# AdamStelmaszczyk/Distributed-BA3C

Measured on AMD Instinct MI355X. Metric: BA3C train-step samples/sec, 84x84x4 frames, batch 32 & 2048, at 1/2/4/8 GPUs, higher is better.
Workload: dtype f32; 1 GPU; configs[2]/[3]: BA3C train step (fwd+bwd+clip+Adam) B=2048/GPU, fc_neurons=512, fc_splits=1, A=4; global_batch=2048, per_gpu_batch=2048, fc_neurons=512, fc_splits=1, num_actions=4, parallelism=dp1, backup_workers=0

## Files before the change

distributed-ba3c_amd/csrc/ba3c_capi.hip:

```cpp
#include <hip/hip_runtime.h>
#include <dlfcn.h>
#include <rccl/rccl.h>

#include <cmath>
#include <cstdio>
#include <cstring>
#include <optional>
#include <string>
#include <type_traits>
#include <vector>

#include "../../include/ba3c.h"
#include "ba3c_band6.h"
#include "ba3c_boxing.h"
#include "ba3c_breakout.h"
#include "ba3c_conv.h"
#include "ba3c_conv3.h"
#include "ba3c_duel.h"
#include "ba3c_envview.h"
#include "ba3c_gemm6.h"
#include "ba3c_launch.h"
#include "ba3c_multi.h"
#include "ba3c_plan.h"
#include "ba3c_problems.h"
// ... 800 lines not shown
                                                          dim3(B * C2D::G::NBANDS), wa, wg, 0, dim3(0, 1, 1), h,
                                                          BA3C_K_CONV2_DGRAD)));
    }
    h->merged[BA3C_K_CONV2_DGRAD] |= 1u << BA3C_K_CONV2_WGRAD;
    return reduce_wgrad6<W2>(h, wa, (int)wg.x, dW2);
  }

  int conv1() {
    if (!pl.split) {
      const WgradPlan p = plan_wgrad(800, 32, B * 1296, 128, 32);
      ConvWgrad<false, 40, 40, 32, 5, 5, 32, true> g{w.p0, w.dp1, w.c1, w.part_1, 1.0f, p.M, p.N, p.K, p.kchunk};
      CHECK((launch_gemm<128, 32, 4, 1>(h, ws, BA3C_K_CONV1_WGRAD, g, p.S)));
      CHECK(conv_reduce(p.M, p.N, p.S, 1, 32, 32, w.part_1));
      ConvDgrad<40, 40, 32, 5, 5, 32, true> d{w.dp1, w.c1, param(h->idx_conv[1]), w.dp0, B * 1600, 32, 800, 0};
      return launch_gemm<128, 32, 4, 1>(h, s, BA3C_K_CONV1_DGRAD, d, 1);
    }
    const Wg6Args wa = wa1();
    float* dW1 = grad(h->idx_conv[1]);
    const int P = pl.conv1_slabs;
    const BandArgs ba{w.dp1, w.c1, w.wt + WT_C1D, w.dp0, nullptr, nullptr, B};
    const SplitIO io{AM_DP1, WJ_C1D, AM_DP0};
    if (pl.mj) {
      CHECK((launch_multi<true, Band6Job<typename LY::C1D>, Wg6Job<W1>>(
          s, band6_args<typename LY::C1D>(h, ba, w, WT_C1D, io), dim3(B * LY::C1D::G::NBANDS), wa,
          wgrad6_grid<W1>(P, B))));
      h->merged[BA3C_K_CONV1_DGRAD] |= 1u << BA3C_K_CONV1_WGRAD;
      return reduce_wgrad6<W1>(h, wa, P, dW1);
    }
    if (pl.conv1_wgrad == Conv1Wgrad::whole) {
      {
        ProbeScope ps(h, ws, BA3C_K_CONV1_WGRAD);
        hipLaunchKernelGGL(wgrad6w_kernel<typename LY::W1W>, dim3(P), dim3(256), 0, ws, wa);
      }
      HIP_TRY(hipGetLastError());
      CHECK(reduce_wgrad6<W1>(h, wa, P, dW1));
    } else if (pl.conv1_wgrad == Conv1Wgrad::wgrad6) {
      CHECK(launch_wgrad6<W1>(h, ws, BA3C_K_CONV1_WGRAD, wa, P, dW1));
    }
    return launch_band6<typename LY::C1D>(h, s, BA3C_K_CONV1_DGRAD, ba, w, WT_C1D, io, pl.ring_dgrad);
  }

  int conv0() {
    ReduceMap mp{};
    mp.kind = 0;
    mp.N = 32;
    mp.cin = CH;
    mp.cinpad = 16;
    mp.dst = grad(h->idx_conv[0]);
    if (pl.split && CH == 4) {
      const int P = pl.conv0_slabs;
      const Conv0WArgs a0{state, w.dp0, w.c0, w.part0, B, w.am(AM_DP0, h)};
      if (pl.conv1_wgrad == Conv1Wgrad::pair0) {
        const Wg6Args wa = wa1();
        {
          ProbeScope ps(h, s, BA3C_K_CONV0_WGRAD);
          HIP_TRY(launch_wgrad01_pair(s, wa, pl.conv1_slabs, a0, P));
        }
        h->merged[BA3C_K_CONV0_WGRAD] |= 1u << BA3C_K_CONV1_WGRAD;
        CHECK(reduce_wgrad6<W1>(h, wa, pl.conv1_slabs, grad(h->idx_conv[1])));
      } else {
        ProbeScope ps(h, s, BA3C_K_CONV0_WGRAD);
        HIP_TRY(launch_conv0s_wgrad(dim3(P), s, a0));
      }
      mp.M = Conv0W<2>::M;
      return add_reduce(h, w.part0, P, mp);
    }
    const WgradPlan p = plan_wgrad(25 * CH, 32, B * 6400, 128, 32);
    ConvWgrad<true, 84, 84, CH, 5, 5, 32, true> g{state, w.dp0, w.c0, w.part0, 1.0f / 255.0f, p.M, p.N, p.K, p.kchunk};
    CHECK((launch_gemm<128, 32, 4, 1>(h, s, BA3C_K_CONV0_WGRAD, g, p.S)));
    mp.M = p.M;
    return add_reduce(h, w.part0, p.S, mp);
  }
};

struct PpoArgs {
  const float* rows;
  float* ratio;
  float clip_eps;
  bool ext = false;
  float vclip_eps = 0.f;
  unsigned flags = 0;
};

template <int LOSS>
void launch_heads(hipStream_t s, int B, const HeadsArgsOf<LOSS>& a) {
  const int F = a.F;
  const dim3 g((B + 3) / 4), t(256);
  if (a.A == 4 && F <= 128 && F > 64) hipLaunchKernelGGL((heads_kernel<2, FC_SPLIT, 4, LOSS>), g, t, 0, s, a);
  else if (a.A == 4 && F <= 512 && F > 256) hipLaunchKernelGGL((heads_kernel<8, FC_SPLIT, 4, LOSS>), g, t, 0, s, a);
  else if (F <= 64) hipLaunchKernelGGL((heads_kernel<1, FC_SPLIT, 0, LOSS>), g, t, 0, s, a);
  else if (F <= 128) hipLaunchKernelGGL((heads_kernel<2, FC_SPLIT, 0, LOSS>), g, t, 0, s, a);
  else if (F <= 256) hipLaunchKernelGGL((heads_kernel<4, FC_SPLIT, 0, LOSS>), g, t, 0, s, a);
  else if (F <= 512) hipLaunchKernelGGL((heads_kernel<8, FC_SPLIT, 0, LOSS>), g, t, 0, s, a);
  else hipLaunchKernelGGL((heads_kernel<0, FC_SPLIT, 0, LOSS>), g, t, 0, s, a);
}

int run_heads(ba3c_handle* h, hipStream_t s, const float* prm, const Workspace& w, int B,
              const int64_t* action, const float* R, float beta, float explore, bool train,
              float* probs, float* probsT, float* value, double* scalars = nullptr,
              bool defer_scalars = false, const PpoArgs* ppo = nullptr) {
  HeadsArgsPpoExt a{};
  if (ppo) {
    a.rows = reinterpret_cast<const float4*>(ppo->rows);
    a.ratio = ppo->ratio;
    a.clip_eps = ppo->clip_eps;
    a.vclip_eps = ppo->vclip_eps;
    a.flags = ppo->flags;
  }
  a.fcpart = w.fcpart;
// ... 142 lines not shown
}

template <class Rules>
static int env_view(void* stream, const int32_t* game, int32_t n_envs, const int32_t* sel, int32_t n_sel,
                    const uint8_t* palette, const uint8_t* hud, int32_t scale, uint8_t* out) {
  if (!game || !palette || !out) return fail(BA3C_ERR_INVALID, "null game / palette / out pointer");
  if (n_envs < 1 || n_sel < 1) return fail(BA3C_ERR_INVALID, "n_envs and n_sel must be >= 1");
  if (scale < 1 || scale > VIEW_MAX_SCALE) return fail(BA3C_ERR_INVALID, "scale must be in [1, 8]");
  if (!check_ptr(game) || ((reinterpret_cast<uintptr_t>(out) | reinterpret_cast<uintptr_t>(sel) |
                            reinterpret_cast<uintptr_t>(hud)) & 3))
    return fail(BA3C_ERR_INVALID, "game must be 16-byte and sel / hud / out 4-byte aligned");
  hipStream_t s = static_cast<hipStream_t>(stream);
  ViewArgs a{game, n_envs, sel, palette, hud, scale, out};
  hipLaunchKernelGGL(env_view_kernel<Rules>, dim3(n_sel), dim3(256), 0, s, a);
  HIP_TRY(hipGetLastError());
  return BA3C_OK;
}

extern "C" {

int ba3c_version(void) { return 1; }

const char* ba3c_last_error(void) { return g_err.c_str(); }

int ba3c_create(const ba3c_config* cfg, ba3c_handle** out) {
  if (!cfg || !out) return fail(BA3C_ERR_INVALID, "null argument");
  const ba3c_config& c = *cfg;
  if (c.channels != 4 && c.channels != 12)
    return fail(BA3C_ERR_INVALID, "channels must be 4 or 12 (FRAME_HISTORY * --channels)");
  if (c.num_actions < 1 || c.num_actions >= MAXA)
    return fail(BA3C_ERR_INVALID, "num_actions must be in [1, 31]");
  if (c.max_batch < 1 || c.max_batch > kMaxBatch)
    return fail(BA3C_ERR_INVALID, "max_batch must be in [1, 16384]");
  const int splits = c.replace_with_conv ? c.fc_splits : c.ps;
  if (splits < 1 || c.fc_neurons < 4 || c.fc_neurons % splits != 0 || (c.fc_neurons / splits) % 4 != 0)
    return fail(BA3C_ERR_INVALID, "fc_neurons must be a multiple of 4*fc_splits (or 4*ps)");
  Switches sw;
  struct Switch {
    const char* name;
    const char* digits;
    void (*set)(Switches&, int);
  };
  const Switch switches[] = {
      {"BA3C_GENERIC", "01", [](Switches& w, int v) { w.generic = v != 0; }},
      {"BA3C_C1PAIR", "02", [](Switches& w, int v) { w.c1pair = v; }},
      {"BA3C_SCALARS_RIDE", "01", [](Switches& w, int v) { w.scalars_ride = v != 0; }},
      {"BA3C_OVERLAP", "012", [](Switches& w, int v) { w.overlap = v; }},
      {"BA3C_MULTI", "01", [](Switches& w, int v) { w.multi = v != 0; }},
      {"BA3C_MULTI_BIG", "0123", [](Switches& w, int v) { w.multi_big = v; }},
      {"BA3C_FUSED_UPDATE", "01", [](Switches& w, int v) { w.fused_update = v != 0; }},
      {"BA3C_RING", "01", [](Switches& w, int v) { w.ring = v != 0; }},
      {"BA3C_CHAIN", "01", [](Switches& w, int v) { w.chain = v != 0; }},
      {"BA3C_FWD01", "01", [](Switches& w, int v) { w.fwd01 = v != 0; }},
  };
  for (const Switch& k : switches) {
    const char* e = getenv(k.name);
    if (!e) continue;
    if (!e[0] || e[1] || !strchr(k.digits, e[0]))
      return fail(BA3C_ERR_INVALID, std::string(k.name) + "=" + e + ": expected one digit of " + k.digits);
    k.set(sw, e[0] - '0');
  }
  ba3c_handle* h = new ba3c_handle();
  h->cfg = c;
  h->sw = sw;
  h->band = h->g6 = !sw.generic;
  {
    int dev = 0, n = 0;
    if (hipGetDevice(&dev) == hipSuccess &&
        hipDeviceGetAttribute(&n, hipDeviceAttributeMultiprocessorCount, dev) == hipSuccess && n > 0)
      h->cus = n;
  }

  const int F = c.fc_neurons, per = F / splits;
  h->per = per;
  int64_t off = 0;
  auto add = [&](const std::string& name, std::initializer_list<int> shape) {
    TensorDesc d;
    d.name = name;
    d.offset = off;
    d.ndim = (int)shape.size();
    int64_t n = 1;
    int i = 0;
    for (int v : shape) {
      d.shape[i++] = v;
      n *= v;
    }
    for (; i < 4; ++i) d.shape[i] = 0;
    d.numel = n;
    h->tensors.push_back(d);
    off = align64(off + n);
    return (int)h->tensors.size() - 1;
  };
  h->idx_conv[0] = add("conv0/W", {5, 5, 16, 32});
  h->idx_conv[1] = add("conv1/W", {5, 5, 32, 32});
  h->idx_conv[2] = add("conv2/W", {5, 5, 32, 64});
  h->idx_conv[3] = add("conv3/W", {3, 3, 64, 64});
  h->idx_fc1 = -1;
  for (int i = 0; i < splits; ++i) {
    int t;
    if (c.replace_with_conv) {
      t = add("fc1_" + std::to_string(i) + "/W", {5, 5, 64, per});
    } else {
      t = add("fc1_" + std::to_string(i) + "/W", {1600, per});
      add("fc1_" + std::to_string(i) + "/b", {per});
    }
    if (i == 0) h->idx_fc1 = t;
// ... 685 lines not shown
```

distributed-ba3c_amd/csrc/ba3c_conv0.hip:

```cpp
#include <hip/hip_runtime.h>

#define BA3C_SHARED_KERNELS 0

#include "ba3c_launch.h"
#include "ba3c_split.h"
#include "ba3c_band6.h"
#include "ba3c_wgrad6.h"

namespace ba3c {

hipError_t launch_conv0s_fwd(dim3 grid, hipStream_t s, const Conv0SArgs& a) {
  hipLaunchKernelGGL(conv0s_fwd_kernel, grid, dim3(256), 0, s, a);
  return hipGetLastError();
}

__global__ void __launch_bounds__(256) __attribute__((amdgpu_waves_per_eu(2)))
wgrad01_pair_kernel(const Wg6Args a1, const Conv0WArgs a0, int g1, int g0) {
  constexpr int B1 = wgrad6w_lds_bytes<Conv1W6W>(), B0 = Conv0W<2>::ALLOC_U4 * 16;
  __shared__ uint4 lds[(B1 > B0 ? B1 : B0) / 16];
  __shared__ uint32_t red4[4];
  const int b = blockIdx.x;
  if (b < g1) {
    wgrad6w_body<Conv1W6W>(a1, b, g1, reinterpret_cast<char*>(lds), red4);
  } else {
    conv0s_wgrad_body<2>(a0, b - g1, g0, lds, red4);
  }
}

hipError_t launch_wgrad01_pair(hipStream_t s, const Wg6Args& a1, int g1, const Conv0WArgs& a0, int g0) {
  hipLaunchKernelGGL(wgrad01_pair_kernel, dim3(g1 + g0), dim3(256), 0, s, a1, a0, g1, g0);
  return hipGetLastError();
}

constexpr int FWD01_CONV0_PRIO = 2;

__device__ __forceinline__ void fwd01_handoff() {
  __builtin_amdgcn_fence(__ATOMIC_RELEASE, "workgroup");
  __syncthreads();
  __builtin_amdgcn_fence(__ATOMIC_ACQUIRE, "workgroup");
}

template <bool TRAIN>
__global__ void __launch_bounds__(256) __attribute__((amdgpu_waves_per_eu(2)))
fwd01_kernel(const Conv0SArgs a0, const Band6Args a1) {
  using L1 = Conv1FLay;
  constexpr int B0 = conv0s_fwd_lds_bytes(), B1 = L1::LDS_BYTES;
  __shared__ uint4 lds4[(B0 > B1 ? B0 : B1) / 16];
  char* lds = reinterpret_cast<char*>(lds4);
  const int gx = gridDim.x, ipw = (a0.batch + gx - 1) / gx;
  const int img0 = min(a0.batch, (int)blockIdx.x * ipw), img1 = min(a0.batch, img0 + ipw);
  constexpr size_t X_IMG = (size_t)Conv0S::HS * Conv0S::WS * Conv0S::C;
  constexpr size_t P0_IMG = (size_t)(Conv0S::HO / 2) * (Conv0S::WO / 2) * Conv0S::COUT;
  constexpr size_t P1_IMG = (size_t)(L1::G::HO / 2) * (L1::G::WO / 2) * L1::G::COUT;
  for (int img = img0; img < img1; ++img) {
    {
      Conv0SArgs s = a0;
      s.x += img * X_IMG;
      s.out += img * P0_IMG;
      if (TRAIN) s.out_code += img * P0_IMG;
      s.amax_out += img;
      s.batch = 1;
      int z = 0;
      asm volatile("" : "+v"(z));
      s.wb += __builtin_amdgcn_readfirstlane(z);
      __builtin_amdgcn_s_setprio(FWD01_CONV0_PRIO);
      conv0s_fwd_body_t<TRAIN, true>(s, 0, 1, lds);
      __builtin_amdgcn_s_setprio(0);
    }
    fwd01_handoff();
    {
      Band6Args s = a1;
      s.src += img * P0_IMG;
      s.out += img * P1_IMG;
      if (TRAIN) s.out_code += img * P1_IMG;
      s.amax_in += img;
      s.amax_out += img;
      s.batch = 1;
      band6r_body<L1, false, true>(s, 0, 1, lds);
    }
    fwd01_handoff();
  }
}

// ... 13 lines not shown
```

distributed-ba3c_amd/csrc/ba3c_launch.h:

```cpp
#pragma once
#include <hip/hip_runtime.h>

namespace ba3c {

struct Conv0SArgs;
struct Conv0WArgs;
struct Wg6Args;
struct Band6Args;

hipError_t launch_conv0s_fwd(dim3 grid, hipStream_t s, const Conv0SArgs& a);
hipError_t launch_fwd01(int grid, hipStream_t s, const Conv0SArgs& a0, const Band6Args& a1);
hipError_t launch_conv0s_wgrad(dim3 grid, hipStream_t s, const Conv0WArgs& a);
hipError_t launch_wgrad01_pair(hipStream_t s, const Wg6Args& a1, int g1, const Conv0WArgs& a0, int g0);

}
```

distributed-ba3c_amd/csrc/ba3c_plan.h:

```cpp
#pragma once
#include <algorithm>

namespace ba3c {

constexpr int SMALL_B = 128;
constexpr int OVERLAP_B = 128;
static_assert(OVERLAP_B <= SMALL_B, "multi-job conv2 input gradient is the small-batch geometry");
constexpr int WG_P1 = 512;
constexpr int W6_P1 = 256, W6_P2 = 128;
constexpr int W1_NBANDS = 9;
constexpr int C0F_NBANDS = 5;
constexpr int C0W_NBANDS = 10;
#ifndef BA3C_C1W_BPW
#define BA3C_C1W_BPW 3
#endif
inline int conv1_wgrad_p(int B) { return std::max(64, std::min(W6_P1, B * W1_NBANDS / BA3C_C1W_BPW)); }
constexpr int W6W_MIN_B = 512, W6W_P = 512;
static_assert(W6W_P <= WG_P1, "conv1 partial slabs: the allocation covers WG_P1 slabs");
inline bool conv1_pair_geometry(int B, int cus) { return B >= 2 * W6W_MIN_B && B % cus == 0 && cus <= WG_P1; }
inline int conv1_w6w_p(int B, int cus) { return conv1_pair_geometry(B, cus) ? cus : std::min(W6W_P, B); }
constexpr int FW_P0S = 512;
inline int conv0_fwd_p(int B) { return std::min(FW_P0S, B * C0F_NBANDS); }
constexpr int C3W_P = 256;
inline int conv3_wgrad_p(int B, int cus) { return std::min(B, std::min(C3W_P, cus)); }
constexpr int WG_P0S = 512;
inline int conv0_wgrad_p(int B, int cus) {
  return conv1_pair_geometry(B, cus) ? cus : std::min(WG_P0S, B * C0W_NBANDS);
}
inline int conv1_slab_count(int B, int cus) {
  return B >= W6W_MIN_B ? conv1_w6w_p(B, cus) : std::min(conv1_wgrad_p(B), B * W1_NBANDS);
}
inline bool ring_batch(int B, int cus) {
  const int pr = 2 * cus;
  return B >= pr && (B % pr == 0 || B >= 8 * pr);
}

struct Switches {
  bool generic = false;
  int c1pair = 2;
  bool scalars_ride = true;
  int overlap = 2;
  bool multi = true;
  int multi_big = 3;
  bool fused_update = true;
  bool ring = true;
  bool chain = true;
  bool fwd01 = true;
};

enum class Conv1Wgrad {
  gemm,
  wgrad6,
  whole,
  pair0,
};

struct LaunchPlan {
  bool split = true;
  bool prep_multi = false;
  bool ring_fwd = false;
  bool fwd01 = false;
  bool conv2_small = false;
  bool big = false;
  bool mj = false;
  bool mj_fc = false;
  bool fc1_big_tiles = false;
  bool mj_c2 = false;
  bool side_stream = false;
  bool ring_dgrad = false;
  Conv1Wgrad conv1_wgrad = Conv1Wgrad::gemm;
  int conv1_slabs = 0, conv0_slabs = 0, conv3_slabs = 0;
};

inline LaunchPlan plan_launches(const Switches& sw, int B, int channels, int cus, bool train) {
  LaunchPlan p;
  p.split = !sw.generic;
  const bool c4 = channels == 4, small = B <= OVERLAP_B, ring = p.split && sw.ring && ring_batch(B, cus);
  p.prep_multi = p.split && sw.multi && small && c4;
  p.ring_fwd = ring;
  p.fwd01 = ring && c4 && !p.prep_multi && sw.fwd01;
  p.conv2_small = p.split && B <= SMALL_B;
  if (!train) return p;
  const bool mjok = p.split && sw.multi && sw.overlap != 1 && c4;
  p.big = !small;
  p.mj = mjok && small;
  p.mj_fc = p.mj || (mjok && (sw.multi_big & 1));
  p.fc1_big_tiles = p.mj_fc && p.big;
  p.mj_c2 = !p.mj && mjok && (sw.multi_big & 2);
  p.side_stream = !p.mj && (sw.overlap == 1 || (sw.overlap == 2 && small));
  p.ring_dgrad = ring;
  if (!p.split) p.conv1_wgrad = Conv1Wgrad::gemm;
  else if (sw.ring && conv1_pair_geometry(B, cus) && sw.c1pair == 2 && c4) p.conv1_wgrad = Conv1Wgrad::pair0;
  else if (B >= W6W_MIN_B) p.conv1_wgrad = Conv1Wgrad::whole;
  else p.conv1_wgrad = Conv1Wgrad::wgrad6;
  p.conv1_slabs = conv1_slab_count(B, cus);
  p.conv0_slabs = c4 ? conv0_wgrad_p(B, cus) : 0;
  p.conv3_slabs = conv3_wgrad_p(B, cus);
  return p;
}

}
```

distributed-ba3c_amd/csrc/ba3c_small.h:

```cpp
#pragma once
#include "ba3c_problems.h"

namespace ba3c {

constexpr int MAXA = 32;
constexpr int NTERMS = 8;
constexpr int MAXT = 48;
constexpr int UPD_CHUNK = 4096;
static_assert(UPD_CHUNK % 256 == 0, "whole elements per thread");
constexpr int FC_SPLIT_MAX = 16;

__device__ __forceinline__ void st_agent(float* p, float v) {
  __hip_atomic_store(p, v, __ATOMIC_RELAXED, __HIP_MEMORY_SCOPE_AGENT);
}
__device__ __forceinline__ float ld_agent(const float* p) {
  return __hip_atomic_load(const_cast<float*>(p), __ATOMIC_RELAXED, __HIP_MEMORY_SCOPE_AGENT);
}
__device__ __forceinline__ unsigned long long ld_agent(const unsigned long long* p) {
  return __hip_atomic_load(const_cast<unsigned long long*>(p), __ATOMIC_RELAXED, __HIP_MEMORY_SCOPE_AGENT);
}

constexpr int LOSS_A3C = 0, LOSS_PPO = 1, LOSS_PPO_EXT = 2;
struct HeadsArgs {
  float* h;
  const float* piW;
  const float* pib;
  const float* vW;
  const float* vb;
  const int64_t* action;
  const float* R;
  float* probs;
  float* probsT;
  float* value;
  float* dzv;
  float* dh;
  float* terms;
  int B, F, A, train, legacy;
  float beta, explore, invB;
  const float* fcpart;
  int fc_split, per, wstride;
  const float* fc_w1;
  unsigned long long* relu_count;
  unsigned long long* done;
  double* scalars;
};
struct HeadsArgsPpo : HeadsArgs {
  const float4* rows;
  float* ratio;
  float clip_eps;
};
constexpr unsigned PPO_ADV_FROM_ROW = 1u;
struct HeadsArgsPpoExt : HeadsArgsPpo {
  float vclip_eps;
  unsigned flags;
// ... 326 lines not shown
    __shared__ int last;
    __builtin_amdgcn_s_waitcnt(0);
    __syncthreads();
    if (threadIdx.x == 0) last = atomicAdd(p.done, 1ull) == (unsigned long long)(nblk - 1);
    __syncthreads();
    if (last) {
      scalars_block(p.terms, p.B, p.beta, p.relu_count, p.scalars);
      if (threadIdx.x == 0) *p.done = 0ull;
    }
  }
}

template <int FCH, int NZ, int AT = 0, int LOSS = LOSS_A3C>
__global__ void __launch_bounds__(256) heads_kernel(const HeadsArgsOf<LOSS> p) {
  heads_body<FCH, NZ, AT, LOSS>(p, blockIdx.x, gridDim.x);
}

__device__ __forceinline__ double block_sum_d(double v, double* red) {
  const int lane = threadIdx.x & 63, wv = threadIdx.x >> 6;
  v = wave_sum_d(v);
  __syncthreads();
  if (lane == 0) red[wv] = v;
  __syncthreads();
  return ((red[0] + red[1]) + red[2]) + red[3];
}

__global__ void __launch_bounds__(256) ppo_norm_adv_kernel(float4* rows, int n, double* stats) {
  __shared__ double red[4];
  const int t = threadIdx.x;
  double s = 0.0;
  for (int i = t; i < n; i += 256) {
    const float4 r = rows[i];
    s += (double)r.x - (double)r.y;
  }
  const double mean = block_sum_d(s, red) / (double)n;
  double q = 0.0;
  for (int i = t; i < n; i += 256) {
    const float4 r = rows[i];
    const double d = ((double)r.x - (double)r.y) - mean;
    q += d * d;
  }
  const double sd = sqrt(block_sum_d(q, red) / (double)n);
  const double inv = sd + 1e-8;
  for (int i = t; i < n; i += 256) {
    const float4 r = rows[i];
    reinterpret_cast<float*>(rows + i)[3] = (float)((((double)r.x - (double)r.y) - mean) / inv);
  }
  if (stats && t == 0) {
    stats[0] = mean;
    stats[1] = sd;
  }
}

struct ReduceMap {
  int kind;
  int M, N;
  int cin, cinpad;
  int per, wstride;
  int A;
  float* dst;
  float* dst_pib;
  float* dst_vW;
  float* dst_vb;
};

__device__ __forceinline__ void grad_store(float* p, float v) { *p = v; }

__device__ __forceinline__ void reduce_store(const ReduceMap& mp, int m, int n, float v) {
  if (mp.kind == 0) {
    const int kk = m / mp.cin, c = m - kk * mp.cin;
    grad_store(mp.dst + ((size_t)kk * mp.cinpad + c) * mp.N + n, v);
  } else if (mp.kind == 1) {
    const int s = n / mp.per, fl = n - s * mp.per;
    grad_store(mp.dst + (size_t)s * mp.wstride + (size_t)m * mp.per + fl, v);
  } else {
    const int F = mp.M - 1;
    if (m < F) {
      if (n < mp.A) grad_store(mp.dst + (size_t)m * mp.A + n, v);
      else if (n == mp.A) grad_store(mp.dst_vW + m, v);
    } else {
      if (n < mp.A) grad_store(mp.dst_pib + n, v);
      else if (n == mp.A) grad_store(mp.dst_vb, v);
    }
  }
}

#ifndef BA3C_RED_GROUPS
#define BA3C_RED_GROUPS 4
#endif
constexpr int RED_G = BA3C_RED_GROUPS;
static_assert(RED_G >= 1 && RED_G <= 16, "reduction groups");

template <int NG>
__device__ __forceinline__ float red_sum(const float (*red)[64], int lane) {
  float v = red[0][lane];
#pragma unroll
  for (int z = 1; z < NG; ++z) v += red[z][lane];
  return v;
}

__global__ void __launch_bounds__(64 * RED_G) wgrad_reduce_kernel(const float* __restrict__ part, int S,
                                                                  const ReduceMap mp) {
  __shared__ float red[RED_G][64];
  const int lane = threadIdx.x & 63, zg = threadIdx.x >> 6;
  const int MN = mp.M * mp.N;
  const int o = blockIdx.x * 64 + lane;
  float s = 0.f;
  if (o < MN) {
    int z = zg;
    for (; z + 7 * RED_G < S; z += 8 * RED_G) {
      float a[8];
#pragma unroll
      for (int u = 0; u < 8; ++u) a[u] = part[(size_t)(z + RED_G * u) * MN + o];
#pragma unroll
      for (int u = 0; u < 8; ++u) s += a[u];
    }
    for (; z < S; z += RED_G) s += part[(size_t)z * MN + o];
  }
  red[zg][lane] = s;
  __syncthreads();
  if (zg == 0 && o < MN) reduce_store(mp, o / mp.N, o % mp.N, red_sum<RED_G>(red, lane));
}

constexpr int MAX_RJOBS = 8;
struct ReduceJobs {
  int n;
  const float* part[MAX_RJOBS];
  int S[MAX_RJOBS];
  ReduceMap mp[MAX_RJOBS];
  int blk0[MAX_RJOBS + 1];
  int vec[MAX_RJOBS];
};

__host__ __device__ inline bool reduce_vec_ok(const ReduceMap& mp) {
  return mp.kind != 2 && mp.N % 4 == 0 && (mp.kind == 0 || mp.per % 4 == 0);
}

__device__ __forceinline__ int reduce_out_size(const ReduceMap& mp) {
  return mp.kind == 0 ? (mp.M / mp.cin) * mp.cinpad * mp.N : mp.M * mp.N;
}

template <int NG>
__device__ __forceinline__ void wgrad_reduce_body(const ReduceJobs& jobs, int b, char* lds) {
  float4 (*red4)[64] = reinterpret_cast<float4 (*)[64]>(lds);
  float (*red)[64] = reinterpret_cast<float (*)[64]>(lds);
  int j = 0;
  while (j + 1 < jobs.n && jobs.blk0[j + 1] <= b) ++j;
  const ReduceMap& mp = jobs.mp[j];
  const float* __restrict__ part = jobs.part[j];
  const int S = jobs.S[j];
  const int lane = threadIdx.x & 63, zg = threadIdx.x >> 6;
  const int MN = mp.M * mp.N;
  if (jobs.vec[j]) {
    const int o = ((b - jobs.blk0[j]) * 64 + lane) * 4;
    const int NO = reduce_out_size(mp);
    int po = o;
    if (mp.kind == 0 && mp.cinpad != mp.cin && o < NO) {
      const int n = o % mp.N, r = o / mp.N, kk = r / mp.cinpad, c = r - kk * mp.cinpad;
      po = c < mp.cin ? (kk * mp.cin + c) * mp.N + n : -1;
    }
    float4 sv = make_float4(0.f, 0.f, 0.f, 0.f);
    if (o < NO && po >= 0) {
      const float4* __restrict__ p4 = reinterpret_cast<const float4*>(part);
      const int MN4 = MN / 4, q = po / 4;
      int z = zg;
      for (; z + 7 * NG < S; z += 8 * NG) {
        float4 a[8];
#pragma unroll
        for (int u = 0; u < 8; ++u) a[u] = p4[(size_t)(z + NG * u) * MN4 + q];
#pragma unroll
        for (int u = 0; u < 8; ++u) {
          sv.x += a[u].x;
          sv.y += a[u].y;
          sv.z += a[u].z;
          sv.w += a[u].w;
        }
      }
      for (; z < S; z += NG) {
        const float4 a = p4[(size_t)z * MN4 + q];
        sv.x += a.x;
        sv.y += a.y;
        sv.z += a.z;
        sv.w += a.w;
      }
    }
    red4[zg][lane] = sv;
    __syncthreads();
    if (zg == 0 && o < NO) {
      float4 v = red4[0][lane];
#pragma unroll
      for (int z = 1; z < NG; ++z) {
        const float4 r = red4[z][lane];
        v.x += r.x;
        v.y += r.y;
        v.z += r.z;
        v.w += r.w;
      }
      if (po < 0) v = make_float4(0.f, 0.f, 0.f, 0.f);
      float* dst;
      if (mp.kind == 0) {
        dst = mp.dst + o;
      } else {
        const int m = o / mp.N, n = o % mp.N, sidx = n / mp.per, fl = n - sidx * mp.per;
        dst = mp.dst + (size_t)sidx * mp.wstride + (size_t)m * mp.per + fl;
      }
      *reinterpret_cast<float4*>(dst) = v;
    }
    return;
  }
  const int o = (b - jobs.blk0[j]) * 64 + lane;
  const int NO = reduce_out_size(mp);
  int po = o;
  if (mp.kind == 0 && mp.cinpad != mp.cin && o < NO) {
    const int n = o % mp.N, r = o / mp.N, kk = r / mp.cinpad, c = r - kk * mp.cinpad;
    po = c < mp.cin ? (kk * mp.cin + c) * mp.N + n : -1;
  }
  float s = 0.f;
  if (o < NO && po >= 0) {
    int z = zg;
    for (; z + 7 * NG < S; z += 8 * NG) {
      float a[8];
#pragma unroll
      for (int u = 0; u < 8; ++u) a[u] = part[(size_t)(z + NG * u) * MN + po];
#pragma unroll
      for (int u = 0; u < 8; ++u) s += a[u];
    }
    for (; z < S; z += NG) s += part[(size_t)z * MN + po];
  }
  red[zg][lane] = s;
  __syncthreads();
  if (zg == 0 && o < NO) {
    const float v = red_sum<NG>(red, lane);
    if (mp.kind == 0) grad_store(mp.dst + o, po >= 0 ? v : 0.f);
    else reduce_store(mp, o / mp.N, o % mp.N, v);
  }
}

__global__ void __launch_bounds__(64 * RED_G) wgrad_reduce_all_kernel(const ReduceJobs jobs) {
  __shared__ float4 red4[RED_G][64];
  wgrad_reduce_body<RED_G>(jobs, blockIdx.x, reinterpret_cast<char*>(red4));
}

struct TensorTable {
  int n;
  int nchunks;
  long long off[MAXT];
  int numel[MAXT];
  int chunk0[MAXT + 1];
};

__device__ __forceinline__ int table_find(const TensorTable& tt, int b) {
  int lo = 0, hi = tt.n - 1;
  while (lo < hi) {
    const int mid = (lo + hi + 1) >> 1;
    if (tt.chunk0[mid] <= b) lo = mid;
    else hi = mid - 1;
  }
  return lo;
}

__device__ __forceinline__ float block_sum_256(float v, float* red) {
  v = wave_sum_f(v);
  const int w = threadIdx.x >> 6;
  if ((threadIdx.x & 63) == 0) red[w] = v;
  __syncthreads();
  const float r = (red[0] + red[1]) + (red[2] + red[3]);
  __syncthreads();
  return r;
}

__global__ void __launch_bounds__(256) sumsq_kernel(const float* __restrict__ g, const TensorTable tt,
                                                    float* __restrict__ part, int cbase) {
  __shared__ float red[4];
  const int b = blockIdx.x + cbase;
  const int t = table_find(tt, b);
  const int c = b - tt.chunk0[t];
  const int beg = c * UPD_CHUNK;
  const int end = min(tt.numel[t], beg + UPD_CHUNK);
  const float* gt = g + tt.off[t];
  float s = 0.f;
  for (int i = beg + threadIdx.x; i < end; i += 256) s = fmaf(gt[i], gt[i], s);
  s = block_sum_256(s, red);
  if (threadIdx.x == 0) part[b] = s;
}

__device__ __forceinline__ float clip_factor(const TensorTable& tt, int t, const float* part) {
  float ss = 0.f;
  for (int b = tt.chunk0[t] + (int)(threadIdx.x & 63); b < tt.chunk0[t + 1]; b += 64) ss += part[b];
// ... 349 lines not shown
```

Measured before the change: 1.223 million samples/s.

## Ride pending wgrad partial reductions as extra workgroups in the conv0/conv1 wgrad pair launch

Already-queued split-K partial-sum reduction jobs (rjobs) are run inside the conv0/conv1 wgrad pair kernel, using one extra workgroup per CU, instead of in a later separate reduce launch. The pending job list is emptied so it is not reduced twice. The riders use new multi-block vectorized reduce bodies that sum several output blocks per workgroup with deeper unrolling. The aim is to drop a kernel launch and hide reduction bandwidth behind the compute-bound wgrad work, at the cost of extra workgroups competing with the pair kernel for CUs and LDS. This relies on the queued jobs' partial buffers being ready before the launch, which holds on the same stream.

After: 1.229 million samples/s (median of 6 runs). No clear change (+0.5%).

```diff
diff --git a/distributed-ba3c_amd/csrc/ba3c_capi.hip b/distributed-ba3c_amd/csrc/ba3c_capi.hip
--- a/distributed-ba3c_amd/csrc/ba3c_capi.hip
+++ b/distributed-ba3c_amd/csrc/ba3c_capi.hip
@@ -876,9 +876,12 @@
       const Conv0WArgs a0{state, w.dp0, w.c0, w.part0, B, w.am(AM_DP0, h)};
       if (pl.conv1_wgrad == Conv1Wgrad::pair0) {
         const Wg6Args wa = wa1();
+        const ReduceJobs ride = h->rjobs;
+        const int gr = pl.reduce_ride && ws == s && ride.n ? h->cus : 0;
+        if (gr) h->rjobs.n = 0;
         {
           ProbeScope ps(h, s, BA3C_K_CONV0_WGRAD);
-          HIP_TRY(launch_wgrad01_pair(s, wa, pl.conv1_slabs, a0, P));
+          HIP_TRY(launch_wgrad01_pair(s, wa, pl.conv1_slabs, a0, P, &ride, gr));
         }
         h->merged[BA3C_K_CONV0_WGRAD] |= 1u << BA3C_K_CONV1_WGRAD;
         CHECK(reduce_wgrad6<W1>(h, wa, pl.conv1_slabs, grad(h->idx_conv[1])));
@@ -1127,6 +1130,7 @@
       {"BA3C_RING", "01", [](Switches& w, int v) { w.ring = v != 0; }},
       {"BA3C_CHAIN", "01", [](Switches& w, int v) { w.chain = v != 0; }},
       {"BA3C_FWD01", "01", [](Switches& w, int v) { w.fwd01 = v != 0; }},
+      {"BA3C_REDUCE_RIDE", "01", [](Switches& w, int v) { w.reduce_ride = v != 0; }},
   };
   for (const Switch& k : switches) {
     const char* e = getenv(k.name);
diff --git a/distributed-ba3c_amd/csrc/ba3c_conv0.hip b/distributed-ba3c_amd/csrc/ba3c_conv0.hip
--- a/distributed-ba3c_amd/csrc/ba3c_conv0.hip
+++ b/distributed-ba3c_amd/csrc/ba3c_conv0.hip
@@ -3,6 +3,7 @@
 #define BA3C_SHARED_KERNELS 0
 
 #include "ba3c_launch.h"
+#include "ba3c_reduce.h"
 #include "ba3c_split.h"
 #include "ba3c_band6.h"
 #include "ba3c_wgrad6.h"
@@ -14,21 +15,62 @@
   return hipGetLastError();
 }
 
+static_assert(64 * RED_G == 256, "a reduce rider is a workgroup of the pair launch");
+
+constexpr int RIDE_KW = 8, RIDE_UW = 2, RIDE_KD = 2, RIDE_UD = 16, RIDE_DEEP_S = 16 * RED_G;
+
+__device__ __forceinline__ int ride_unit_blocks(const ReduceJobs& rj, int j) {
+  return !rj.vec[j] ? 1 : rj.S[j] >= RIDE_DEEP_S ? RIDE_KD : RIDE_KW;
+}
+
+__device__ __forceinline__ void reduce_ride_body(const ReduceJobs& rj, int r, int gr, char* lds) {
+  int total = 0;
+  for (int j = 0; j < rj.n; ++j) {
+    const int kb = ride_unit_blocks(rj, j);
+    total += (rj.blk0[j + 1] - rj.blk0[j] + kb - 1) / kb;
+  }
+  for (int unit = r; unit < total; unit += gr) {
+    int j = rj.n - 1, u = unit, kb, nu;
+    for (;; --j) {
+      kb = ride_unit_blocks(rj, j);
+      nu = (rj.blk0[j + 1] - rj.blk0[j] + kb - 1) / kb;
+      if (u < nu || j == 0) break;
+      u -= nu;
+    }
+    const int b = u * kb, nblk = min(kb, rj.blk0[j + 1] - rj.blk0[j] - b);
+    if (!rj.vec[j]) {
+      wgrad_reduce_body<RED_G>(rj, rj.blk0[j] + b, lds);
+      __syncthreads();
+    } else if (kb == RIDE_KD) {
+      wgrad_reduce_vec_blocks<RED_G, RIDE_KD, RIDE_UD>(rj, j, b, nblk, lds);
+    } else {
+      wgrad_reduce_vec_blocks<RED_G, RIDE_KW, RIDE_UW>(rj, j, b, nblk, lds);
+    }
+  }
+}
+
 __global__ void __launch_bounds__(256) __attribute__((amdgpu_waves_per_eu(2)))
-wgrad01_pair_kernel(const Wg6Args a1, const Conv0WArgs a0, int g1, int g0) {
+wgrad01_pair_kernel(const Wg6Args a1, const Conv0WArgs a0, int g1, int g0, const ReduceJobs rj) {
   constexpr int B1 = wgrad6w_lds_bytes<Conv1W6W>(), B0 = Conv0W<2>::ALLOC_U4 * 16;
+  constexpr int BR = (RIDE_KW > RIDE_KD ? RIDE_KW : RIDE_KD) * RED_G * 64 * (int)sizeof(float4);
+  static_assert(BR <= (B1 > B0 ? B1 : B0), "the riders' scratch fits the pair's LDS array");
   __shared__ uint4 lds[(B1 > B0 ? B1 : B0) / 16];
   __shared__ uint32_t red4[4];
   const int b = blockIdx.x;
   if (b < g1) {
     wgrad6w_body<Conv1W6W>(a1, b, g1, reinterpret_cast<char*>(lds), red4);
+  } else if (b < g1 + g0) {
+    conv0s_wgrad_body<2>(a0, b - g1, g0, lds, red4);
   } else {
-    conv0s_wgrad_body<2>(a0, b - g1, g0, lds, red4);
+    reduce_ride_body(rj, b - g1 - g0, (int)gridDim.x - g1 - g0, reinterpret_cast<char*>(lds));
   }
 }
 
-hipError_t launch_wgrad01_pair(hipStream_t s, const Wg6Args& a1, int g1, const Conv0WArgs& a0, int g0) {
-  hipLaunchKernelGGL(wgrad01_pair_kernel, dim3(g1 + g0), dim3(256), 0, s, a1, a0, g1, g0);
+hipError_t launch_wgrad01_pair(hipStream_t s, const Wg6Args& a1, int g1, const Conv0WArgs& a0, int g0,
+                               const ReduceJobs* rj, int gr) {
+  static const ReduceJobs none{};
+  if (!rj || rj->n == 0) gr = 0;
+  hipLaunchKernelGGL(wgrad01_pair_kernel, dim3(g1 + g0 + gr), dim3(256), 0, s, a1, a0, g1, g0, gr ? *rj : none);
   return hipGetLastError();
 }
 
diff --git a/distributed-ba3c_amd/csrc/ba3c_launch.h b/distributed-ba3c_amd/csrc/ba3c_launch.h
--- a/distributed-ba3c_amd/csrc/ba3c_launch.h
+++ b/distributed-ba3c_amd/csrc/ba3c_launch.h
@@ -7,10 +7,12 @@
 struct Conv0WArgs;
 struct Wg6Args;
 struct Band6Args;
+struct ReduceJobs;
 
 hipError_t launch_conv0s_fwd(dim3 grid, hipStream_t s, const Conv0SArgs& a);
 hipError_t launch_fwd01(int grid, hipStream_t s, const Conv0SArgs& a0, const Band6Args& a1);
 hipError_t launch_conv0s_wgrad(dim3 grid, hipStream_t s, const Conv0WArgs& a);
-hipError_t launch_wgrad01_pair(hipStream_t s, const Wg6Args& a1, int g1, const Conv0WArgs& a0, int g0);
+hipError_t launch_wgrad01_pair(hipStream_t s, const Wg6Args& a1, int g1, const Conv0WArgs& a0, int g0,
+                               const ReduceJobs* rj, int gr);
 
 }
diff --git a/distributed-ba3c_amd/csrc/ba3c_plan.h b/distributed-ba3c_amd/csrc/ba3c_plan.h
--- a/distributed-ba3c_amd/csrc/ba3c_plan.h
+++ b/distributed-ba3c_amd/csrc/ba3c_plan.h
@@ -46,6 +46,7 @@
   bool ring = true;
   bool chain = true;
   bool fwd01 = true;
+  bool reduce_ride = true;
 };
 
 enum class Conv1Wgrad {
@@ -69,6 +70,7 @@
   bool side_stream = false;
   bool ring_dgrad = false;
   Conv1Wgrad conv1_wgrad = Conv1Wgrad::gemm;
+  bool reduce_ride = false;
   int conv1_slabs = 0, conv0_slabs = 0, conv3_slabs = 0;
 };
 
@@ -93,6 +95,7 @@
   else if (sw.ring && conv1_pair_geometry(B, cus) && sw.c1pair == 2 && c4) p.conv1_wgrad = Conv1Wgrad::pair0;
   else if (B >= W6W_MIN_B) p.conv1_wgrad = Conv1Wgrad::whole;
   else p.conv1_wgrad = Conv1Wgrad::wgrad6;
+  p.reduce_ride = sw.reduce_ride && p.conv1_wgrad == Conv1Wgrad::pair0 && !p.side_stream;
   p.conv1_slabs = conv1_slab_count(B, cus);
   p.conv0_slabs = c4 ? conv0_wgrad_p(B, cus) : 0;
   p.conv3_slabs = conv3_wgrad_p(B, cus);
diff --git a/distributed-ba3c_amd/csrc/ba3c_reduce.h b/distributed-ba3c_amd/csrc/ba3c_reduce.h
--- /dev/null
+++ b/distributed-ba3c_amd/csrc/ba3c_reduce.h
@@ -0,0 +1,246 @@
+#pragma once
+#include <hip/hip_runtime.h>
+
+namespace ba3c {
+
+struct ReduceMap {
+  int kind;
+  int M, N;
+  int cin, cinpad;
+  int per, wstride;
+  int A;
+  float* dst;
+  float* dst_pib;
+  float* dst_vW;
+  float* dst_vb;
+};
+
+__device__ __forceinline__ void grad_store(float* p, float v) { *p = v; }
+
+__device__ __forceinline__ void reduce_store(const ReduceMap& mp, int m, int n, float v) {
+  if (mp.kind == 0) {
+    const int kk = m / mp.cin, c = m - kk * mp.cin;
+    grad_store(mp.dst + ((size_t)kk * mp.cinpad + c) * mp.N + n, v);
+  } else if (mp.kind == 1) {
+    const int s = n / mp.per, fl = n - s * mp.per;
+    grad_store(mp.dst + (size_t)s * mp.wstride + (size_t)m * mp.per + fl, v);
+  } else {
+    const int F = mp.M - 1;
+    if (m < F) {
+      if (n < mp.A) grad_store(mp.dst + (size_t)m * mp.A + n, v);
+      else if (n == mp.A) grad_store(mp.dst_vW + m, v);
+    } else {
+      if (n < mp.A) grad_store(mp.dst_pib + n, v);
+      else if (n == mp.A) grad_store(mp.dst_vb, v);
+    }
+  }
+}
+
+#ifndef BA3C_RED_GROUPS
+#define BA3C_RED_GROUPS 4
+#endif
+constexpr int RED_G = BA3C_RED_GROUPS;
+static_assert(RED_G >= 1 && RED_G <= 16, "reduction groups");
+
+template <int NG>
+__device__ __forceinline__ float red_sum(const float (*red)[64], int lane) {
+  float v = red[0][lane];
+#pragma unroll
+  for (int z = 1; z < NG; ++z) v += red[z][lane];
+  return v;
+}
+
+constexpr int MAX_RJOBS = 8;
+struct ReduceJobs {
+  int n;
+  const float* part[MAX_RJOBS];
+  int S[MAX_RJOBS];
+  ReduceMap mp[MAX_RJOBS];
+  int blk0[MAX_RJOBS + 1];
+  int vec[MAX_RJOBS];
+};
+
+__host__ __device__ inline bool reduce_vec_ok(const ReduceMap& mp) {
+  return mp.kind != 2 && mp.N % 4 == 0 && (mp.kind == 0 || mp.per % 4 == 0);
+}
+
+__device__ __forceinline__ int reduce_out_size(const ReduceMap& mp) {
+  return mp.kind == 0 ? (mp.M / mp.cin) * mp.cinpad * mp.N : mp.M * mp.N;
+}
+
+template <int NG>
+__device__ __forceinline__ void wgrad_reduce_body(const ReduceJobs& jobs, int b, char* lds) {
+  float4 (*red4)[64] = reinterpret_cast<float4 (*)[64]>(lds);
+  float (*red)[64] = reinterpret_cast<float (*)[64]>(lds);
+  int j = 0;
+  while (j + 1 < jobs.n && jobs.blk0[j + 1] <= b) ++j;
+  const ReduceMap& mp = jobs.mp[j];
+  const float* __restrict__ part = jobs.part[j];
+  const int S = jobs.S[j];
+  const int lane = threadIdx.x & 63, zg = threadIdx.x >> 6;
+  const int MN = mp.M * mp.N;
+  if (jobs.vec[j]) {
+    const int o = ((b - jobs.blk0[j]) * 64 + lane) * 4;
+    const int NO = reduce_out_size(mp);
+    int po = o;
+    if (mp.kind == 0 && mp.cinpad != mp.cin && o < NO) {
+      const int n = o % mp.N, r = o / mp.N, kk = r / mp.cinpad, c = r - kk * mp.cinpad;
+      po = c < mp.cin ? (kk * mp.cin + c) * mp.N + n : -1;
+    }
+    float4 sv = make_float4(0.f, 0.f, 0.f, 0.f);
+    if (o < NO && po >= 0) {
+      const float4* __restrict__ p4 = reinterpret_cast<const float4*>(part);
+      const int MN4 = MN / 4, q = po / 4;
+      int z = zg;
+      for (; z + 7 * NG < S; z += 8 * NG) {
+        float4 a[8];
+#pragma unroll
+        for (int u = 0; u < 8; ++u) a[u] = p4[(size_t)(z + NG * u) * MN4 + q];
+#pragma unroll
+        for (int u = 0; u < 8; ++u) {
+          sv.x += a[u].x;
+          sv.y += a[u].y;
+          sv.z += a[u].z;
+          sv.w += a[u].w;
+        }
+      }
+      for (; z < S; z += NG) {
+        const float4 a = p4[(size_t)z * MN4 + q];
+        sv.x += a.x;
+        sv.y += a.y;
+        sv.z += a.z;
+        sv.w += a.w;
+      }
+    }
+    red4[zg][lane] = sv;
+    __syncthreads();
+    if (zg == 0 && o < NO) {
+      float4 v = red4[0][lane];
+#pragma unroll
+      for (int z = 1; z < NG; ++z) {
+        const float4 r = red4[z][lane];
+        v.x += r.x;
+        v.y += r.y;
+        v.z += r.z;
+        v.w += r.w;
+      }
+      if (po < 0) v = make_float4(0.f, 0.f, 0.f, 0.f);
+      float* dst;
+      if (mp.kind == 0) {
+        dst = mp.dst + o;
+      } else {
+        const int m = o / mp.N, n = o % mp.N, sidx = n / mp.per, fl = n - sidx * mp.per;
+        dst = mp.dst + (size_t)sidx * mp.wstride + (size_t)m * mp.per + fl;
+      }
+      *reinterpret_cast<float4*>(dst) = v;
+    }
+    return;
+  }
+  const int o = (b - jobs.blk0[j]) * 64 + lane;
+  const int NO = reduce_out_size(mp);
+  int po = o;
+  if (mp.kind == 0 && mp.cinpad != mp.cin && o < NO) {
+    const int n = o % mp.N, r = o / mp.N, kk = r / mp.cinpad, c = r - kk * mp.cinpad;
+    po = c < mp.cin ? (kk * mp.cin + c) * mp.N + n : -1;
+  }
+  float s = 0.f;
+  if (o < NO && po >= 0) {
+    int z = zg;
+    for (; z + 7 * NG < S; z += 8 * NG) {
+      float a[8];
+#pragma unroll
+      for (int u = 0; u < 8; ++u) a[u] = part[(size_t)(z + NG * u) * MN + po];
+#pragma unroll
+      for (int u = 0; u < 8; ++u) s += a[u];
+    }
+    for (; z < S; z += NG) s += part[(size_t)z * MN + po];
+  }
+  red[zg][lane] = s;
+  __syncthreads();
+  if (zg == 0 && o < NO) {
+    const float v = red_sum<NG>(red, lane);
+    if (mp.kind == 0) grad_store(mp.dst + o, po >= 0 ? v : 0.f);
+    else reduce_store(mp, o / mp.N, o % mp.N, v);
+  }
+}
+
+template <int NG, int K, int U>
+__device__ __forceinline__ void wgrad_reduce_vec_blocks(const ReduceJobs& jobs, int j, int b, int nblk, char* lds) {
+  float4 (*red4)[NG][64] = reinterpret_cast<float4 (*)[NG][64]>(lds);
+  const ReduceMap& mp = jobs.mp[j];
+  const float4* __restrict__ p4 = reinterpret_cast<const float4*>(jobs.part[j]);
+  const int S = jobs.S[j];
+  const int lane = threadIdx.x & 63, zg = threadIdx.x >> 6;
+  const int MN4 = mp.M * mp.N / 4, NO = reduce_out_size(mp);
+  int q[K];
+#pragma unroll
+  for (int k = 0; k < K; ++k) {
+    const int o = ((b + k) * 64 + lane) * 4;
+    int po = o;
+    if (mp.kind == 0 && mp.cinpad != mp.cin && o < NO) {
+      const int n = o % mp.N, r = o / mp.N, kk = r / mp.cinpad, c = r - kk * mp.cinpad;
+      po = c < mp.cin ? (kk * mp.cin + c) * mp.N + n : -1;
+    }
+    q[k] = k < nblk && o < NO && po >= 0 ? po / 4 : 0;
+  }
+  float4 sv[K];
+#pragma unroll
+  for (int k = 0; k < K; ++k) sv[k] = make_float4(0.f, 0.f, 0.f, 0.f);
+  int z = zg;
+  for (; z + (U - 1) * NG < S; z += U * NG) {
+    float4 a[K][U];
+#pragma unroll
+    for (int u = 0; u < U; ++u)
+#pragma unroll
+      for (int k = 0; k < K; ++k) a[k][u] = p4[(size_t)(z + NG * u) * MN4 + q[k]];
+#pragma unroll
+    for (int k = 0; k < K; ++k)
+#pragma unroll
+      for (int u = 0; u < U; ++u) {
+        sv[k].x += a[k][u].x;
+        sv[k].y += a[k][u].y;
+        sv[k].z += a[k][u].z;
+        sv[k].w += a[k][u].w;
+      }
+  }
+  for (; z < S; z += NG) {
+    float4 a[K];
+#pragma unroll
+    for (int k = 0; k < K; ++k) a[k] = p4[(size_t)z * MN4 + q[k]];
+#pragma unroll
+    for (int k = 0; k < K; ++k) {
+      sv[k].x += a[k].x;
+      sv[k].y += a[k].y;
+      sv[k].z += a[k].z;
+      sv[k].w += a[k].w;
+    }
+  }
+#pragma unroll
+  for (int k = 0; k < K; ++k) red4[k][zg][lane] = sv[k];
+  __syncthreads();
+  for (int k = zg; k < nblk; k += NG) {
+    const int o = ((b + k) * 64 + lane) * 4;
+    if (o >= NO) continue;
+    float4 v = red4[k][0][lane];
+#pragma unroll
+    for (int g = 1; g < NG; ++g) {
+      const float4 r = red4[k][g][lane];
+      v.x += r.x;
+      v.y += r.y;
+      v.z += r.z;
+      v.w += r.w;
+    }
+    float* dst;
+    if (mp.kind == 0) {
+      dst = mp.dst + o;
+      if (mp.cinpad != mp.cin && (o / mp.N) % mp.cinpad >= mp.cin) v = make_float4(0.f, 0.f, 0.f, 0.f);
+    } else {
+      const int m = o / mp.N, n = o % mp.N, sidx = n / mp.per, fl = n - sidx * mp.per;
+      dst = mp.dst + (size_t)sidx * mp.wstride + (size_t)m * mp.per + fl;
+    }
+    *reinterpret_cast<float4*>(dst) = v;
+  }
+  __syncthreads();
+}
+
+}
diff --git a/distributed-ba3c_amd/csrc/ba3c_small.h b/distributed-ba3c_amd/csrc/ba3c_small.h
--- a/distributed-ba3c_amd/csrc/ba3c_small.h
+++ b/distributed-ba3c_amd/csrc/ba3c_small.h
@@ -1,5 +1,6 @@
 #pragma once
 #include "ba3c_problems.h"
+#include "ba3c_reduce.h"
 
 namespace ba3c {
 
@@ -432,53 +433,6 @@
   }
 }
 
-struct ReduceMap {
-  int kind;
-  int M, N;
-  int cin, cinpad;
-  int per, wstride;
-  int A;
-  float* dst;
-  float* dst_pib;
-  float* dst_vW;
-  float* dst_vb;
-};
-
-__device__ __forceinline__ void grad_store(float* p, float v) { *p = v; }
-
-__device__ __forceinline__ void reduce_store(const ReduceMap& mp, int m, int n, float v) {
-  if (mp.kind == 0) {
-    const int kk = m / mp.cin, c = m - kk * mp.cin;
-    grad_store(mp.dst + ((size_t)kk * mp.cinpad + c) * mp.N + n, v);
-  } else if (mp.kind == 1) {
-    const int s = n / mp.per, fl = n - s * mp.per;
-    grad_store(mp.dst + (size_t)s * mp.wstride + (size_t)m * mp.per + fl, v);
-  } else {
-    const int F = mp.M - 1;
-    if (m < F) {
-      if (n < mp.A) grad_store(mp.dst + (size_t)m * mp.A + n, v);
-      else if (n == mp.A) grad_store(mp.dst_vW + m, v);
-    } else {
-      if (n < mp.A) grad_store(mp.dst_pib + n, v);
-      else if (n == mp.A) grad_store(mp.dst_vb, v);
-    }
-  }
-}
-
-#ifndef BA3C_RED_GROUPS
-#define BA3C_RED_GROUPS 4
-#endif
-constexpr int RED_G = BA3C_RED_GROUPS;
-static_assert(RED_G >= 1 && RED_G <= 16, "reduction groups");
-
-template <int NG>
-__device__ __forceinline__ float red_sum(const float (*red)[64], int lane) {
-  float v = red[0][lane];
-#pragma unroll
-  for (int z = 1; z < NG; ++z) v += red[z][lane];
-  return v;
-}
-
 __global__ void __launch_bounds__(64 * RED_G) wgrad_reduce_kernel(const float* __restrict__ part, int S,
                                                                   const ReduceMap mp) {
   __shared__ float red[RED_G][64];
@@ -500,120 +454,6 @@
   red[zg][lane] = s;
   __syncthreads();
   if (zg == 0 && o < MN) reduce_store(mp, o / mp.N, o % mp.N, red_sum<RED_G>(red, lane));
-}
-
-constexpr int MAX_RJOBS = 8;
-struct ReduceJobs {
-  int n;
-  const float* part[MAX_RJOBS];
-  int S[MAX_RJOBS];
-  ReduceMap mp[MAX_RJOBS];
-  int blk0[MAX_RJOBS + 1];
-  int vec[MAX_RJOBS];
-};
-
-__host__ __device__ inline bool reduce_vec_ok(const ReduceMap& mp) {
-  return mp.kind != 2 && mp.N % 4 == 0 && (mp.kind == 0 || mp.per % 4 == 0);
-}
-
-__device__ __forceinline__ int reduce_out_size(const ReduceMap& mp) {
-  return mp.kind == 0 ? (mp.M / mp.cin) * mp.cinpad * mp.N : mp.M * mp.N;
-}
-
-template <int NG>
-__device__ __forceinline__ void wgrad_reduce_body(const ReduceJobs& jobs, int b, char* lds) {
-  float4 (*red4)[64] = reinterpret_cast<float4 (*)[64]>(lds);
-  float (*red)[64] = reinterpret_cast<float (*)[64]>(lds);
-  int j = 0;
-  while (j + 1 < jobs.n && jobs.blk0[j + 1] <= b) ++j;
-  const ReduceMap& mp = jobs.mp[j];
-  const float* __restrict__ part = jobs.part[j];
-  const int S = jobs.S[j];
-  const int lane = threadIdx.x & 63, zg = threadIdx.x >> 6;
-  const int MN = mp.M * mp.N;
-  if (jobs.vec[j]) {
-    const int o = ((b - jobs.blk0[j]) * 64 + lane) * 4;
-    const int NO = reduce_out_size(mp);
-    int po = o;
-    if (mp.kind == 0 && mp.cinpad != mp.cin && o < NO) {
-      const int n = o % mp.N, r = o / mp.N, kk = r / mp.cinpad, c = r - kk * mp.cinpad;
-      po = c < mp.cin ? (kk * mp.cin + c) * mp.N + n : -1;
-    }
-    float4 sv = make_float4(0.f, 0.f, 0.f, 0.f);
-    if (o < NO && po >= 0) {
-      const float4* __restrict__ p4 = reinterpret_cast<const float4*>(part);
-      const int MN4 = MN / 4, q = po / 4;
-      int z = zg;
-      for (; z + 7 * NG < S; z += 8 * NG) {
-        float4 a[8];
-#pragma unroll
-        for (int u = 0; u < 8; ++u) a[u] = p4[(size_t)(z + NG * u) * MN4 + q];
-#pragma unroll
-        for (int u = 0; u < 8; ++u) {
-          sv.x += a[u].x;
-          sv.y += a[u].y;
-          sv.z += a[u].z;
-          sv.w += a[u].w;
-        }
-      }
-      for (; z < S; z += NG) {
-        const float4 a = p4[(size_t)z * MN4 + q];
-        sv.x += a.x;
-        sv.y += a.y;
-        sv.z += a.z;
-        sv.w += a.w;
-      }
-    }
-    red4[zg][lane] = sv;
-    __syncthreads();
-    if (zg == 0 && o < NO) {
-      float4 v = red4[0][lane];
-#pragma unroll
-      for (int z = 1; z < NG; ++z) {
-        const float4 r = red4[z][lane];
-        v.x += r.x;
-        v.y += r.y;
-        v.z += r.z;
-        v.w += r.w;
-      }
-      if (po < 0) v = make_float4(0.f, 0.f, 0.f, 0.f);
-      float* dst;
-      if (mp.kind == 0) {
-        dst = mp.dst + o;
-      } else {
-        const int m = o / mp.N, n = o % mp.N, sidx = n / mp.per, fl = n - sidx * mp.per;
-        dst = mp.dst + (size_t)sidx * mp.wstride + (size_t)m * mp.per + fl;
-      }
-      *reinterpret_cast<float4*>(dst) = v;
-    }
-    return;
-  }
-  const int o = (b - jobs.blk0[j]) * 64 + lane;
-  const int NO = reduce_out_size(mp);
-  int po = o;
-  if (mp.kind == 0 && mp.cinpad != mp.cin && o < NO) {
-    const int n = o % mp.N, r = o / mp.N, kk = r / mp.cinpad, c = r - kk * mp.cinpad;
-    po = c < mp.cin ? (kk * mp.cin + c) * mp.N + n : -1;
-  }
-  float s = 0.f;
-  if (o < NO && po >= 0) {
-    int z = zg;
-    for (; z + 7 * NG < S; z += 8 * NG) {
-      float a[8];
-#pragma unroll
-      for (int u = 0; u < 8; ++u) a[u] = part[(size_t)(z + NG * u) * MN + po];
-#pragma unroll
-      for (int u = 0; u < 8; ++u) s += a[u];
-    }
-    for (; z < S; z += NG) s += part[(size_t)z * MN + po];
-  }
-  red[zg][lane] = s;
-  __syncthreads();
-  if (zg == 0 && o < NO) {
-    const float v = red_sum<NG>(red, lane);
-    if (mp.kind == 0) grad_store(mp.dst + o, po >= 0 ? v : 0.f);
-    else reduce_store(mp, o / mp.N, o % mp.N, v);
-  }
 }
 
 __global__ void __launch_bounds__(64 * RED_G) wgrad_reduce_all_kernel(const ReduceJobs jobs) {
```
